# dist1ll/pomcpp

Measured on NVIDIA B200. Metric: env-steps/sec, higher is better.
Workload: dtype u8/int32

## Files before the change

pomcpp_b200/csrc/pom_batch.cu:

```cuda
#include <cuda_runtime.h>
#include <cstdio>
#include <cstdlib>
#include <cstring>
#include <fstream>
#include <sched.h>
#include <string>
#include <vector>
#include <new>

#include "pom_batch.h"
#include "pom_kernels.cuh"

namespace
{

thread_local std::string g_err;

int fail(int code, const char* what, cudaError_t ce = cudaSuccess)
{
    g_err = what;
    if(ce != cudaSuccess)
    {
        g_err += ": ";
        g_err += cudaGetErrorString(ce);
// ... 9 lines not shown
};

#define CK(expr) do { cudaError_t ce_ = (expr); if(ce_ != cudaSuccess) return fail(POM_E_CUDA, #expr, ce_); } while(0)

constexpr uint64_t TILE_ALIGN = 256;
constexpr uint64_t XFER_CHUNK = 65536;
constexpr size_t   FLUSH_BYTES = size_t(256) << 20;

}

struct pom_batch {
    int       device = 0;
    uint64_t  n_envs = 0;
    uint64_t  n_alloc = 0;
    uint64_t  env_offset = 0;
    uint32_t  n_templates = 0;
    uint32_t  max_ticks = 0;
    int       tpb = 128;
    int       n_sms = 1;
    int       ws_nw = 20;
    uint32_t  attr_ws = 0;
    uint32_t  walk = 0;
    int       pingpong = 1;
    int       no_spec = 0;
    int       policy_pertick = 1;
    int       obs_fused = 0;
    int       step_kernel = 0;
    bool      teams = false;
    int       policy_view = -1;
    uint8_t*  recs = nullptr;
    uint8_t*  templates = nullptr;
    uint32_t* episodes = nullptr;
    unsigned long long* stats = nullptr;
    uint32_t* moves_buf = nullptr;
    uint8_t*  status_buf = nullptr;
    pom_state* aos_stage = nullptr;
    uint8_t*  st_stage = nullptr;
    uint32_t* bad_count = nullptr;
    uint32_t* fin_counter = nullptr;
    uint32_t* policy = nullptr;
    void*     flush_buf = nullptr;
    uint32_t* idx_buf = nullptr;
    uint64_t  idx_cap = 0;
    cudaEvent_t ev_expand = nullptr;
    cudaStream_t stream = nullptr;
    cudaEvent_t ev[2] = { nullptr, nullptr };
    static constexpr int MAX_CHUNKS = 16;
    cudaStream_t s_h2d = nullptr, s_d2h = nullptr, s_k2 = nullptr;
    cudaEvent_t ev_k2 = nullptr;
    cudaEvent_t ev_in[MAX_CHUNKS] = {}, ev_done[MAX_CHUNKS] = {}, ev_out = nullptr, ev_begin = nullptr;
    std::vector<int32_t> seeds;
    uint64_t  launches = 0;
    bool      forked = false;
    uint32_t  attr_done = 0;

    pomk::BatchParams params() const
    {
        pomk::BatchParams P;
        P.recs = recs; P.n_envs = n_envs; P.env_offset = env_offset; P.templates = templates;
        P.n_templates = n_templates; P.max_ticks = max_ticks;
        P.tmpl_mask = (n_templates & (n_templates - 1u)) == 0u ? n_templates - 1u : 0u; P.episodes = episodes; P.stats = stats;
        P.policy = policy; P.policy_stride = n_alloc;
        return P;
    }
};

namespace
{

int use(const pom_batch* cb, bool join = true)
{
    if(!cb) return fail(POM_E_ARG, "null handle");
    CK(cudaSetDevice(cb->device));
    pom_batch* b = const_cast<pom_batch*>(cb);
    if(join && b->forked)
    {
        CK(cudaEventRecord(b->ev_k2, b->s_k2));
        CK(cudaStreamWaitEvent(b->stream, b->ev_k2, 0));
        b->forked = false;
    }
    return POM_OK;
}

enum { ATTR_STEP = 1, ATTR_ROLLOUT = 2, ATTR_ROLLOUT_POLICY = 4, ATTR_POLICY_MOVES = 8, ATTR_EXPAND = 16, ATTR_OBS = 32, ATTR_ROLLOUT_SPEC = 64, ATTR_OBS_CROPPED = 128 };
constexpr uint32_t attr_bit(uint32_t which, bool teams, bool fog = false) { return (fog ? which << 16 : which) << (teams ? 8 : 0); }

uint32_t policy_view_bits(const pom_batch* b)
{
    return uint32_t(b->policy_view > 15 ? 15 : b->policy_view) << pomk::POLICY_VIEW_SHIFT;
}

template<typename K>
int set_smem(pom_batch* b, uint32_t which, K kernel, uint32_t bytes)
{
    if(b->attr_done & which) return POM_OK;
    CK(cudaFuncSetAttribute(kernel, cudaFuncAttributeMaxDynamicSharedMemorySize, int(bytes)));
    b->attr_done |= which;
    return POM_OK;
}

int ensure_stage(pom_batch* b)
{
    if(!b->aos_stage)
    {
        CK(cudaMalloc(&b->aos_stage, XFER_CHUNK * sizeof(pom_state)));
        CK(cudaMalloc(&b->st_stage, XFER_CHUNK));
        CK(cudaMalloc(&b->bad_count, sizeof(uint32_t)));
    }
    return POM_OK;
}

int ensure_policy(pom_batch* b)
{
    if(!b->policy)
    {
        CK(cudaMalloc(&b->policy, 9 * b->n_alloc * sizeof(uint32_t)));
        CK(cudaMemsetAsync(b->policy, 0, 9 * b->n_alloc * sizeof(uint32_t), b->stream));
    }
    return POM_OK;
}

int fill_from_templates(pom_batch* b)
{
    const uint64_t words = b->n_envs * POM_REC_WORDS;
    pomk::k_fill_from_templates<<<unsigned((words + 255) / 256), 256, 0, b->stream>>>(b->params());
    b->launches++;
    CK(cudaGetLastError());
// ... 31 lines not shown
            b->launches++;
            CK(cudaGetLastError());
            CK(cudaStreamSynchronize(b->stream));
            b->seeds.resize(n);
            for(uint32_t k = 0; k < n; k++) b->seeds[k] = first_seed + int32_t(idx[k]);
            return POM_OK;
        }
    }
    return fail(POM_E_ARG, "could not find enough clean seeds");
}

int pack_into(pom_batch* b, uint8_t* dst_recs, uint64_t first, uint64_t count, const pom_state* states, const uint8_t* status, uint32_t* bad_total)
{
    int rc = ensure_stage(b);
    if(rc) return rc;
    for(uint64_t done = 0; done < count; done += XFER_CHUNK)
    {
        const uint64_t c = count - done < XFER_CHUNK ? count - done : XFER_CHUNK;
        CK(cudaMemcpyAsync(b->aos_stage, states + done, c * sizeof(pom_state), cudaMemcpyHostToDevice, b->stream));
        if(status) CK(cudaMemcpyAsync(b->st_stage, status + done, c, cudaMemcpyHostToDevice, b->stream));
        CK(cudaMemsetAsync(b->bad_count, 0, sizeof(uint32_t), b->stream));
        pomk::k_pack<<<unsigned((c + 127) / 128), 128, 0, b->stream>>>(b->aos_stage, status ? b->st_stage : nullptr, dst_recs, first + done, c, b->bad_count);
        b->launches++;
        CK(cudaGetLastError());
        uint32_t bad = 0;
        CK(cudaMemcpyAsync(&bad, b->bad_count, sizeof(uint32_t), cudaMemcpyDeviceToHost, b->stream));
        CK(cudaStreamSynchronize(b->stream));
        *bad_total += bad;
    }
    return POM_OK;
}

constexpr int WS_NW = 20, WS_NBUF = 24;

template<int NW, bool OBS, bool FREEZE = false, bool SPEC = false, bool TEAMS = false>
int launch_step_ws(pom_batch* b, const pomk::BatchParams& P, const pomk::StepIO& io, uint32_t flags, cudaStream_t on)
{
    typedef pomk::RingScratch<WS_NBUF> R;
    const uint32_t bit = TEAMS ? (1u << (24 + (FREEZE ? 2 : (OBS ? 1 : 0)))) :
                         SPEC ? 2u : (FREEZE ? 1u : (1u << (NW + (OBS ? 1 : 0))));
    if(!(b->attr_ws & bit))
    {
        CK(cudaFuncSetAttribute(pomk::k_step_ws<NW, WS_NBUF, OBS, FREEZE, SPEC, TEAMS>, cudaFuncAttributeMaxDynamicSharedMemorySize, int(R::BYTES)));
        b->attr_ws |= bit;
    }
    const uint64_t n_slices = (P.n_envs + 31) / 32;
    const unsigned grid = unsigned(n_slices < uint64_t(b->n_sms) ? n_slices : uint64_t(b->n_sms));
    pomk::k_step_ws<NW, WS_NBUF, OBS, FREEZE, SPEC, TEAMS><<<grid, (NW + 1) * 32, R::BYTES, on ? on : b->stream>>>(P, io, flags);
    b->launches++;
    CK(cudaGetLastError());
    return POM_OK;
}

int launch_step_io(pom_batch* b, const pomk::BatchParams& P, pomk::StepIO io, uint32_t flags, cudaStream_t on)
{
    io.bulk = (reinterpret_cast<uintptr_t>(io.moves) & 15u) == 0u ? 1u : 0u;
    if(P.n_envs == b->n_envs && b->pingpong) io.reverse = (b->walk++) & 1u;
    if(b->teams)
    {
        if(flags & pomk::STEP_FREEZE_TRUNCATED) return launch_step_ws<WS_NW, false, true, false, true>(b, P, io, flags, on);
        if(io.obs) return launch_step_ws<WS_NW, true, false, false, true>(b, P, io, flags, on);
        return launch_step_ws<WS_NW, false, false, false, true>(b, P, io, flags, on);
    }
    if(flags & pomk::STEP_FREEZE_TRUNCATED) return launch_step_ws<WS_NW, false, true>(b, P, io, flags, on);
    if(b->ws_nw == WS_NW && (flags & ~uint32_t(POM_STEP_OVERLAP)) == uint32_t(POM_STEP_AUTORESET | POM_STEP_COUNT) && io.bulk &&
       !io.status_out && !io.obs && !io.joint && !io.done_bits && !io.fin_env && !b->no_spec)
        return launch_step_ws<WS_NW, false, false, true>(b, P, io, flags, on);
    if(io.obs) return launch_step_ws<WS_NW, true>(b, P, io, flags, on);
    switch(b->ws_nw)
    {
    case 12: return launch_step_ws<12, false>(b, P, io, flags, on);
    case 14: return launch_step_ws<14, false>(b, P, io, flags, on);
    case 16: return launch_step_ws<16, false>(b, P, io, flags, on);
    case 18: return launch_step_ws<18, false>(b, P, io, flags, on);
    case 22: return launch_step_ws<22, false>(b, P, io, flags, on);
    default: return launch_step_ws<WS_NW, false>(b, P, io, flags, on);
    }
}

template<int TPB, bool TEAMS = false>
int launch_step(pom_batch* b, const uint8_t* moves_dev, uint32_t flags, uint8_t* status_dev, uint64_t first = 0, uint64_t count = 0, cudaStream_t on = nullptr,
                bool tile_kernel = false)
{
    pomk::BatchParams P = b->params();
    if(count)
    {
        P.recs += first * POM_REC_BYTES; P.episodes += first; P.env_offset += first; P.n_envs = count;
        moves_dev += 4 * first;
        if(status_dev) status_dev += first;
    }
    if(b->step_kernel == 0 && !tile_kernel)
    {
        pomk::StepIO io{};
        io.moves = moves_dev;
        io.status_out = status_dev;
        return launch_step_io(b, P, io, flags, on);
    }
    { int rc = set_smem(b, attr_bit(ATTR_STEP, TEAMS), pomk::k_step<TPB, TEAMS>, pomk::TileScratch<TPB>::BYTES); if(rc) return rc; }
    const unsigned grid = unsigned((P.n_envs + TPB - 1) / TPB);
    pomk::k_step<TPB, TEAMS><<<grid, TPB, pomk::TileScratch<TPB>::BYTES, on ? on : b->stream>>>(P, reinterpret_cast<const uint32_t*>(moves_dev), flags, status_dev);
    b->launches++;
    CK(cudaGetLastError());
    return POM_OK;
}

template<int TPB, bool TEAMS = false, bool FOG = false>
// ... 121 lines not shown
    } while(0)
#define POM_DISPATCH_MODE(h, fn, ...) \
    do { \
        if((h)->teams) return fn<128, true>(__VA_ARGS__); \
        POM_DISPATCH(h, fn, __VA_ARGS__); \
    } while(0)
#define POM_DISPATCH_POLICY(h, fn, ...) \
    do { \
        if((h)->policy_view >= 0) \
        { \
            if((h)->teams) return fn<128, true, true>(__VA_ARGS__); \
            return fn<128, false, true>(__VA_ARGS__); \
        } \
        POM_DISPATCH_MODE(h, fn, __VA_ARGS__); \
    } while(0)

extern "C" {

const char* pom_last_error(void) { return g_err.c_str(); }

int pom_device_count(void)
{
    int n = 0;
    if(cudaGetDeviceCount(&n) != cudaSuccess) { cudaGetLastError(); return 0; }
    return n;
}

int pom_batch_init(pom_batch** out, int device, uint64_t n_envs, const pom_init_desc* desc)
{
    if(!out || !desc || n_envs == 0 || desc->n_templates == 0) return fail(POM_E_ARG, "pom_batch_init: bad argument");
    if(n_envs > (uint64_t(1) << 31)) return fail(POM_E_ARG, "pom_batch_init: too many envs for one handle");
    int ndev = 0;
    cudaError_t ce = cudaGetDeviceCount(&ndev);
    if(ce != cudaSuccess || ndev == 0) return fail(POM_E_CUDA, "no CUDA device: the step path has no CPU fallback", ce);
    if(device < 0 || device >= ndev) return fail(POM_E_ARG, "pom_batch_init: no such device");
    CK(cudaSetDevice(device));
    pom_batch* b = new(std::nothrow) pom_batch();
    if(!b) return fail(POM_E_NOMEM, "host allocation failed");
    b->device = device;
    b->n_envs = n_envs;
    b->n_alloc = (n_envs + TILE_ALIGN - 1) / TILE_ALIGN * TILE_ALIGN;
    b->env_offset = desc->env_offset;
    b->n_templates = desc->n_templates;
    b->max_ticks = desc->max_ticks;
    b->teams = (desc->flags & POM_INIT_TEAMS) != 0;
    cudaDeviceGetAttribute(&b->n_sms, cudaDevAttrMultiProcessorCount, device);
    if(b->n_sms < 1) b->n_sms = 1;
    if(const char* e = std::getenv("POM_STEP_KERNEL")) b->step_kernel = std::strcmp(e, "tile") == 0 ? 1 : 0;
    if(const char* e = std::getenv("POM_WS_NW")) b->ws_nw = std::atoi(e);
    if(const char* e = std::getenv("POM_STEP_PINGPONG")) b->pingpong = std::atoi(e) != 0;
    if(const char* e = std::getenv("POM_OBS_FUSED")) b->obs_fused = std::atoi(e) != 0;
    if(const char* e = std::getenv("POM_WS_NOSPEC")) b->no_spec = std::atoi(e) != 0;
    if(const char* e = std::getenv("POM_ROLL_POLICY")) b->policy_pertick = std::strcmp(e, "fused") != 0;
    if(const char* e = std::getenv("POM_TPB"))
    {
        const int t = std::atoi(e);
        if(t == 32 || t == 64 || t == 128 || t == 256) b->tpb = t;
    }
    int rc = POM_OK;
    do {
        if(cudaStreamCreateWithFlags(&b->stream, cudaStreamNonBlocking) != cudaSuccess ||
           cudaEventCreate(&b->ev[0]) != cudaSuccess || cudaEventCreate(&b->ev[1]) != cudaSuccess ||
           cudaStreamCreateWithFlags(&b->s_h2d, cudaStreamNonBlocking) != cudaSuccess ||
           cudaStreamCreateWithFlags(&b->s_d2h, cudaStreamNonBlocking) != cudaSuccess ||
           cudaStreamCreateWithFlags(&b->s_k2, cudaStreamNonBlocking) != cudaSuccess ||
           cudaEventCreateWithFlags(&b->ev_k2, cudaEventDisableTiming) != cudaSuccess ||
           cudaEventCreateWithFlags(&b->ev_out, cudaEventDisableTiming) != cudaSuccess ||
           cudaEventCreateWithFlags(&b->ev_begin, cudaEventDisableTiming) != cudaSuccess)
        { rc = fail(POM_E_CUDA, "stream/event creation failed", cudaGetLastError()); break; }
        if(cudaMalloc(&b->recs, b->n_alloc * POM_REC_BYTES) != cudaSuccess ||
           cudaMalloc(&b->templates, size_t(b->n_templates) * POM_REC_BYTES) != cudaSuccess ||
           cudaMalloc(&b->episodes, b->n_alloc * sizeof(uint32_t)) != cudaSuccess ||
           cudaMalloc(&b->stats, POM_STATS_WORDS * sizeof(unsigned long long)) != cudaSuccess ||
           cudaMalloc(&b->moves_buf, b->n_alloc * 4) != cudaSuccess ||
           cudaMalloc(&b->status_buf, b->n_alloc) != cudaSuccess)
        { rc = fail(POM_E_NOMEM, "device allocation failed", cudaGetLastError()); break; }
        if(cudaMemsetAsync(b->recs, 0, b->n_alloc * POM_REC_BYTES, b->stream) != cudaSuccess ||
           cudaMemsetAsync(b->episodes, 0, b->n_alloc * sizeof(uint32_t), b->stream) != cudaSuccess ||
           cudaMemsetAsync(b->stats, 0, POM_STATS_WORDS * sizeof(unsigned long long), b->stream) != cudaSuccess)
        { rc = fail(POM_E_CUDA, "memset failed", cudaGetLastError()); break; }
        if(desc->host_templates)
        {
            uint32_t bad = 0;
            rc = pack_into(b, b->templates, 0, b->n_templates, desc->host_templates, nullptr, &bad);
            if(rc) break;
            if(bad) { rc = fail(POM_E_STATE, "a host template cannot be represented in the packed record"); break; }
        }
        else
        {
            rc = build_templates_from_seeds(b, desc->first_seed);
            if(rc) break;
        }
        if(!(desc->flags & POM_INIT_EMPTY))
        {
            rc = fill_from_templates(b);
            if(rc) break;
        }
        if(cudaStreamSynchronize(b->stream) != cudaSuccess) { rc = fail(POM_E_CUDA, "init sync failed", cudaGetLastError()); break; }
    } while(0);
    if(rc) { pom_batch_destroy(b); return rc; }
    *out = b;
    return POM_OK;
}

int pom_batch_destroy(pom_batch* b)
{
    if(!b) return POM_OK;
    cudaSetDevice(b->device);
    if(b->s_k2) cudaStreamSynchronize(b->s_k2);
    if(b->stream) cudaStreamSynchronize(b->stream);
    cudaFree(b->recs); cudaFree(b->templates); cudaFree(b->episodes); cudaFree(b->stats);
    cudaFree(b->moves_buf); cudaFree(b->status_buf); cudaFree(b->aos_stage); cudaFree(b->st_stage);
    cudaFree(b->bad_count); cudaFree(b->flush_buf); cudaFree(b->idx_buf); if(b->ev_expand) cudaEventDestroy(b->ev_expand); cudaFree(b->policy); cudaFree(b->fin_counter);
    if(b->ev[0]) cudaEventDestroy(b->ev[0]);
    if(b->ev[1]) cudaEventDestroy(b->ev[1]);
    for(int i = 0; i < pom_batch::MAX_CHUNKS; i++) { if(b->ev_in[i]) cudaEventDestroy(b->ev_in[i]); if(b->ev_done[i]) cudaEventDestroy(b->ev_done[i]); }
    if(b->ev_out) cudaEventDestroy(b->ev_out);
    if(b->ev_begin) cudaEventDestroy(b->ev_begin);
    if(b->s_h2d) cudaStreamDestroy(b->s_h2d);
    if(b->s_d2h) cudaStreamDestroy(b->s_d2h);
    if(b->s_k2) cudaStreamDestroy(b->s_k2);
    if(b->ev_k2) cudaEventDestroy(b->ev_k2);
    if(b->stream) cudaStreamDestroy(b->stream);
    delete b;
    return POM_OK;
}

int pom_batch_sync(pom_batch* b)
{
    int rc = use(b); if(rc) return rc;
    CK(cudaStreamSynchronize(b->stream));
    return POM_OK;
}

int pom_batch_upload(pom_batch* b, uint64_t first, uint64_t count, const pom_state* states, const uint8_t* status)
{
    int rc = use(b); if(rc) return rc;
    if(!states) return fail(POM_E_ARG, "pom_batch_upload: null states");
    if(first > b->n_envs || count > b->n_envs - first) return fail(POM_E_RANGE, "pom_batch_upload: range outside the batch");
    uint32_t bad = 0;
    rc = pack_into(b, b->recs, first, count, states, status, &bad);
    if(rc) return rc;
    if(bad) return fail(POM_E_STATE, "pom_batch_upload: some states cannot be represented (marked POM_STATUS_INVALID)");
    return POM_OK;
}

int pom_batch_download(pom_batch* b, uint64_t first, uint64_t count, pom_state* states, uint8_t* status)
{
    int rc = use(b); if(rc) return rc;
    if(first > b->n_envs || count > b->n_envs - first) return fail(POM_E_RANGE, "pom_batch_download: range outside the batch");
    rc = ensure_stage(b); if(rc) return rc;
    for(uint64_t done = 0; done < count; done += XFER_CHUNK)
    {
        const uint64_t c = count - done < XFER_CHUNK ? count - done : XFER_CHUNK;
        pomk::k_unpack<<<unsigned((c + 127) / 128), 128, 0, b->stream>>>(b->recs, states ? b->aos_stage : nullptr, b->st_stage, first + done, c);
        b->launches++;
        CK(cudaGetLastError());
        if(states) CK(cudaMemcpyAsync(states + done, b->aos_stage, c * sizeof(pom_state), cudaMemcpyDeviceToHost, b->stream));
        if(status) CK(cudaMemcpyAsync(status + done, b->st_stage, c, cudaMemcpyDeviceToHost, b->stream));
        CK(cudaStreamSynchronize(b->stream));
    }
    return POM_OK;
}

int pom_batch_observe(pom_batch* b, uint64_t first, uint64_t count, int agent, int view, pom_state* states, uint8_t* status)
// ... 17 lines not shown
}

uint64_t pom_batch_obs_stride(const pom_batch* b) { return b ? b->n_alloc : 0; }

int pom_batch_observe_planes(pom_batch* b, uint8_t* obs_dev, uint32_t agent_mask, int view)
{
    int rc = use(b); if(rc) return rc;
    if(!obs_dev) return fail(POM_E_ARG, "pom_batch_observe_planes: null output");
    if(agent_mask == 0 || agent_mask > 0xFu || view < 0) return fail(POM_E_ARG, "pom_batch_observe_planes: agent_mask must be 1..15 and view >= 0");
    POM_DISPATCH(b, launch_observe_planes, b, obs_dev, agent_mask, view);
}

int pom_device_copy(int device, void* dst, const void* src, uint64_t bytes)
{
    if(!dst || !src) return fail(POM_E_ARG, "pom_device_copy: null pointer");
    CK(cudaSetDevice(device));
    CK(cudaMemcpy(dst, src, bytes, cudaMemcpyDefault));
    return POM_OK;
}

int pom_batch_reset(pom_batch* b)
{
    int rc = use(b); if(rc) return rc;
    CK(cudaMemsetAsync(b->episodes, 0, b->n_alloc * sizeof(uint32_t), b->stream));
    CK(cudaMemsetAsync(b->stats, 0, POM_STATS_WORDS * sizeof(unsigned long long), b->stream));
    if(b->policy) CK(cudaMemsetAsync(b->policy, 0, 9 * b->n_alloc * sizeof(uint32_t), b->stream));
    return fill_from_templates(b);
}

int pom_batch_templates(pom_batch* b, pom_state* out, int32_t* seeds_out)
{
    int rc = use(b); if(rc) return rc;
    if(!out) return fail(POM_E_ARG, "pom_batch_templates: null output");
    rc = ensure_stage(b); if(rc) return rc;
    for(uint64_t done = 0; done < b->n_templates; done += XFER_CHUNK)
    {
        const uint64_t c = b->n_templates - done < XFER_CHUNK ? b->n_templates - done : XFER_CHUNK;
        pomk::k_unpack<<<unsigned((c + 127) / 128), 128, 0, b->stream>>>(b->templates, b->aos_stage, b->st_stage, done, c);
        b->launches++;
        CK(cudaGetLastError());
        CK(cudaMemcpyAsync(out + done, b->aos_stage, c * sizeof(pom_state), cudaMemcpyDeviceToHost, b->stream));
        CK(cudaStreamSynchronize(b->stream));
    }
    if(seeds_out)
    {
        for(uint32_t k = 0; k < b->n_templates; k++) seeds_out[k] = k < b->seeds.size() ? b->seeds[k] : 0;
    }
    return POM_OK;
}

int pom_batch_step(pom_batch* b, const uint8_t* moves_dev, uint32_t flags)
{
    const bool overlap = (flags & POM_STEP_OVERLAP) && b && b->n_envs >= (uint64_t(1) << 18);
    int rc = use(b, !overlap); if(rc) return rc;
    if(!moves_dev) return fail(POM_E_ARG, "pom_batch_step: null moves");
    if(!overlap) POM_DISPATCH_MODE(b, launch_step, b, moves_dev, flags, nullptr);
    static int parts = -1;
    if(parts < 0) { const char* e = std::getenv("POM_STEP_PARTS"); parts = e ? std::atoi(e) : 2; if(parts < 2 || parts > 16) parts = 2; }
    const uint64_t per = ((b->n_envs + parts - 1) / parts + 1023) / 1024 * 1024;
    const bool tile_parts = b->n_envs <= (uint64_t(1) << 19) && !b->no_spec;
    CK(cudaEventRecord(b->ev_begin, b->stream));
    CK(cudaStreamWaitEvent(b->s_k2, b->ev_begin, 0));
    int c = 0;
    for(uint64_t first = 0; first < b->n_envs; first += per, c++)
    {
        const uint64_t count = first + per <= b->n_envs ? per : b->n_envs - first;
        rc = [&]() -> int { POM_DISPATCH_MODE(b, launch_step, b, moves_dev, flags, nullptr, first, count, (c & 1) ? b->s_k2 : b->stream, tile_parts); }();
        if(rc) return rc;
    }
    b->forked = true;
    return POM_OK;
}

static int enqueue_step_pipeline(pom_batch* b, const uint8_t* moves_host, uint8_t* status_host, uint32_t flags, int chunks, uint64_t per)
{
    const uint64_t n = b->n_envs;
    CK(cudaEventRecord(b->ev_begin, b->stream));
    CK(cudaStreamWaitEvent(b->s_h2d, b->ev_begin, 0));
    if(chunks > 1) CK(cudaStreamWaitEvent(b->s_k2, b->ev_begin, 0));
    for(int c = 0; c < chunks; c++)
    {
        const uint64_t first = uint64_t(c) * per, count = (first + per <= n) ? per : n - first;
        cudaStream_t compute = (c & 1) ? b->s_k2 : b->stream;
        CK(cudaMemcpyAsync(reinterpret_cast<uint8_t*>(b->moves_buf) + 4 * first, moves_host + 4 * first, 4 * count, cudaMemcpyHostToDevice, b->s_h2d));
        CK(cudaEventRecord(b->ev_in[c], b->s_h2d));
        CK(cudaStreamWaitEvent(compute, b->ev_in[c], 0));
        const int rc = [&]() -> int { POM_DISPATCH_MODE(b, launch_step, b, reinterpret_cast<const uint8_t*>(b->moves_buf), flags,
                                                   status_host ? b->status_buf : nullptr, first, count, compute); }();
        if(rc) return rc;
        if(status_host)
        {
            CK(cudaEventRecord(b->ev_done[c], compute));
            CK(cudaStreamWaitEvent(b->s_d2h, b->ev_done[c], 0));
            CK(cudaMemcpyAsync(status_host + first, b->status_buf + first, count, cudaMemcpyDeviceToHost, b->s_d2h));
        }
    }
    if(chunks > 1)
    {
        CK(cudaEventRecord(b->ev_k2, b->s_k2));
        CK(cudaStreamWaitEvent(b->stream, b->ev_k2, 0));
    }
    if(status_host)
    {
        CK(cudaEventRecord(b->ev_out, b->s_d2h));
        CK(cudaStreamWaitEvent(b->stream, b->ev_out, 0));
    }
    return POM_OK;
}

// ... 488 lines not shown
```

pomcpp_b200/csrc/pom_kernels.cuh:

```cuda
#ifndef POM_KERNELS_CUH_
#define POM_KERNELS_CUH_

#include <cuda_runtime.h>
#include <stdint.h>
#include "pom_core.cuh"
#include "pom_policy.cuh"
#include "pom_batch.h"

namespace pomk
{

constexpr uint32_t STEP_FREEZE_TRUNCATED = 0x40000000u;

enum { ST_STEPS = 0, ST_EPISODES = 1, ST_WIN0 = 2, ST_DRAWS = 6, ST_TRUNC = 7, ST_SUMLEN = 8, ST_INVALID = 9 };

struct BatchParams {
    uint8_t*            recs;
    uint64_t            n_envs;
    uint64_t            env_offset;
    const uint8_t*      templates;
    uint32_t            n_templates;
    uint32_t            tmpl_mask;
    uint32_t            max_ticks;
    uint32_t*           episodes;
// ... 1 lines not shown
    uint32_t*           policy;
    uint64_t            policy_stride;
};

__device__ __forceinline__ uint32_t smem_u32(const void* p) { return uint32_t(__cvta_generic_to_shared(p)); }

__device__ __forceinline__ void mbar_init(uint64_t* bar, uint32_t count)
{
    asm volatile("mbarrier.init.shared::cta.b64 [%0], %1;" :: "r"(smem_u32(bar)), "r"(count));
}
__device__ __forceinline__ void fence_barrier_init()
{
    asm volatile("fence.mbarrier_init.release.cluster;" ::: "memory");
}
__device__ __forceinline__ void fence_proxy_async()
{
    asm volatile("fence.proxy.async.shared::cta;" ::: "memory");
}
__device__ __forceinline__ void mbar_expect_tx(uint64_t* bar, uint32_t bytes)
{
    asm volatile("mbarrier.arrive.expect_tx.shared::cta.b64 _, [%0], %1;" :: "r"(smem_u32(bar)), "r"(bytes) : "memory");
}
__device__ __forceinline__ void mbar_arrive(uint64_t* bar)
{
    asm volatile("mbarrier.arrive.shared::cta.b64 _, [%0];" :: "r"(smem_u32(bar)) : "memory");
}
__device__ __forceinline__ void mbar_wait(uint64_t* bar, uint32_t parity)
{
    asm volatile(
        "{\n"
        ".reg .pred p;\n"
        "WAIT_LOOP:\n"
        "mbarrier.try_wait.parity.shared::cta.b64 p, [%0], %1;\n"
        "@p bra WAIT_DONE;\n"
        "bra WAIT_LOOP;\n"
        "WAIT_DONE:\n"
        "}\n" :: "r"(smem_u32(bar)), "r"(parity) : "memory");
}
__device__ __forceinline__ void bulk_g2s(void* smem_dst, const void* gmem_src, uint32_t bytes, uint64_t* bar)
{
    asm volatile("cp.async.bulk.shared::cluster.global.mbarrier::complete_tx::bytes [%0], [%1], %2, [%3];"
                 :: "r"(smem_u32(smem_dst)), "l"(gmem_src), "r"(bytes), "r"(smem_u32(bar)) : "memory");
}
__device__ __forceinline__ void bulk_s2g(void* gmem_dst, const void* smem_src, uint32_t bytes)
{
    asm volatile("cp.async.bulk.global.shared::cta.bulk_group [%0], [%1], %2;"
                 :: "l"(gmem_dst), "r"(smem_u32(smem_src)), "r"(bytes) : "memory");
    asm volatile("cp.async.bulk.commit_group;" ::: "memory");
}
__device__ __forceinline__ void bulk_wait_read_all()
{
    asm volatile("cp.async.bulk.wait_group.read 0;" ::: "memory");
}

__device__ __forceinline__ void warp_add(unsigned long long* dst, uint32_t v)
{
    const uint32_t s = __reduce_add_sync(0xFFFFFFFFu, v);
    if((threadIdx.x & 31u) == 0u && s) atomicAdd(dst, (unsigned long long)s);
}

struct EpisodeAcc {
    uint32_t fin_draw = 0u;
    uint32_t trunc_abort = 0u;
    uint32_t win01 = 0u, win23 = 0u;
    uint32_t len = 0u;
    uint32_t steps = 0u;
    uint32_t pending = 0u;
};

__device__ __forceinline__ void acc_add(EpisodeAcc& A, bool fin, uint32_t status, uint32_t len)
{
    if(!fin) return;
    const bool done = (status & POM_STATUS_DONE) != 0u;
    const bool draw = done && (status & POM_STATUS_DRAW);
    const bool trunc = !done && (status & POM_STATUS_TRUNCATED);
    const uint32_t w = (status & POM_STATUS_WINNER_MASK) >> POM_STATUS_WINNER_SHIFT;
    A.fin_draw += 1u + (draw ? 0x10000u : 0u);
    A.trunc_abort += (trunc ? 1u : 0u) + ((!done && !trunc) ? 0x10000u : 0u);
    if(done && !draw)
    {
        const uint32_t inc = (w & 1u) ? 0x10000u : 1u;
        if(w & 2u) A.win23 += inc; else A.win01 += inc;
    }
    A.len += len;
    A.pending++;
}

__device__ __forceinline__ void acc_flush(unsigned long long* stats, EpisodeAcc& A, bool count_steps)
{
    const uint32_t lane = threadIdx.x & 31u;
    if(__reduce_or_sync(0xFFFFFFFFu, A.pending))
    {
        const uint32_t v[9] = { A.fin_draw & 0xFFFFu, A.win01 & 0xFFFFu, A.win01 >> 16, A.win23 & 0xFFFFu, A.win23 >> 16,
                                A.fin_draw >> 16, A.trunc_abort & 0xFFFFu, A.len, A.trunc_abort >> 16 };
#pragma unroll
        for(int k = 0; k < 9; k++)
        {
            const uint32_t sum = __reduce_add_sync(0xFFFFFFFFu, v[k]);
            if(lane == 0u && sum) atomicAdd(stats + 1 + k, (unsigned long long)sum);
        }
    }
    if(count_steps)
    {
        const uint32_t sum = __reduce_add_sync(0xFFFFFFFFu, A.steps);
        if(lane == 0u && sum) atomicAdd(stats + ST_STEPS, (unsigned long long)sum);
    }
// ... 203 lines not shown
template<int TPB, bool TEAMS = false>
__global__ void __launch_bounds__(TPB) k_step(BatchParams P, const uint32_t* __restrict__ moves, uint32_t flags, uint8_t* __restrict__ status_out)
{
    extern __shared__ __align__(128) uint8_t smem[];
    const uint64_t env = uint64_t(blockIdx.x) * TPB + threadIdx.x;
    const bool active = env < P.n_envs;
    const bool raw = (flags & POM_STEP_RAW) != 0u;

    constexpr uint32_t SLICE_BYTES = 32 * POM_REC_BYTES;
    const uint32_t warp = threadIdx.x >> 5, lane = threadIdx.x & 31u;
    uint64_t* bar = reinterpret_cast<uint64_t*>(smem + TileScratch<TPB>::OFF_BAR) + warp;
    uint8_t* sslice = smem + warp * SLICE_BYTES;
    uint8_t* gslice = P.recs + (size_t(blockIdx.x) * TPB + warp * 32u) * POM_REC_BYTES;
    if(lane == 0)
    {
        mbar_init(bar, 1);
        fence_barrier_init();
        mbar_expect_tx(bar, SLICE_BYTES);
        bulk_g2s(sslice, gslice, SLICE_BYTES, bar);
    }
    const uint32_t m = active ? __ldg(moves + env) : 0u;
    uint32_t ep_now = (active && (flags & POM_STEP_AUTORESET)) ? P.episodes[env] : 0u;
    __syncwarp();
    mbar_wait(bar, 0);

    uint8_t* rec = sslice + lane * POM_REC_BYTES;
    const bool stepped = active && !(rec[R_STATUS] & (raw ? POM_STATUS_INVALID : (POM_STATUS_DONE | POM_STATUS_INVALID)));
    warp_tick<TEAMS>(sslice, rec, m, stepped, raw, smem + TileScratch<TPB>::OFF_LIST + 8u * warp,
                     (flags & POM_STEP_CONTINUE_UNDEFINED) ? pomcore::F_INVALID_MASK_CONTINUE : pomcore::F_INVALID_MASK);
    EpisodeAcc acc;
    acc.steps = stepped ? 1u : 0u;
    uint32_t st_end = active ? rec[R_STATUS] : 0u;
    if(flags & POM_STEP_AUTORESET)
    {
        const uint32_t st = finish_and_reset(sslice, rec, P, env, active && stepped, true, ep_now, acc);
        if(active && stepped) st_end = st;
    }
    acc_flush(P.stats, acc, (flags & POM_STEP_COUNT) != 0u);
    if(status_out && active) status_out[env] = uint8_t(st_end);
    fence_proxy_async();
    __syncwarp();
    if(lane == 0)
    {
        bulk_s2g(gslice, sslice, SLICE_BYTES);
        bulk_wait_read_all();
    }
}

struct StepIO {
    const void* moves;
    uint32_t    joint;
    uint32_t    bulk;
    uint32_t    reverse;
    uint8_t*    status_out;
    uint32_t*   done_bits;
    uint32_t*   fin_env;
    uint8_t*    fin_status;
    uint32_t*   fin_counter;
    uint32_t*   fin_count_out;
    uint32_t    fin_capacity;
    uint8_t*    obs;
    uint64_t    obs_stride;
    uint32_t    obs_mask;
    int         obs_view;
};

__device__ __forceinline__ uint32_t moves_of_joint(uint32_t j)
{
    const uint32_t a0 = j % 6u, r1 = j / 6u, a1 = r1 % 6u, r2 = r1 / 6u, a2 = r2 % 6u, a3 = (r2 / 6u) % 6u;
    return a0 | (a1 << 8) | (a2 << 16) | (a3 << 24);
}

template<int NBUF> struct RingScratch {
    static constexpr uint32_t SLICE_BYTES = 32 * POM_REC_BYTES;
    static constexpr uint32_t SLOT = SLICE_BYTES + 128 + 16;
    static constexpr uint32_t OFF_FULL = NBUF * SLOT;
    static constexpr uint32_t MAIL = 256;
    static constexpr uint32_t OFF_MAIL = OFF_FULL + 8 * NBUF;
    static constexpr uint32_t OFF_TICKET = OFF_MAIL + 4 * MAIL;
    static constexpr uint32_t FIN_CAP = 480;
    static constexpr uint32_t OFF_FIN = OFF_TICKET + 16;
    static constexpr uint32_t OFF_FIN_ENV = OFF_FIN + 16;
    static constexpr uint32_t OFF_FIN_ST = OFF_FIN_ENV + 4 * FIN_CAP;
    static constexpr uint32_t BYTES = OFF_FIN_ST + FIN_CAP;
};

template<int NW, int NBUF, bool OBS, bool FREEZE, bool SPEC = false, bool TEAMS = false>
__global__ void __launch_bounds__((NW + 1) * 32, 1) k_step_ws(BatchParams P, StepIO io_in, uint32_t flags_in)
{
    const uint32_t flags = SPEC ? uint32_t(POM_STEP_AUTORESET | POM_STEP_COUNT) : flags_in;
    StepIO io = io_in;
    if(SPEC)
    {
        io.joint = 0u; io.bulk = 1u; io.status_out = nullptr; io.obs = nullptr; io.done_bits = nullptr; io.fin_env = nullptr;
    }
    const uint32_t* __restrict__ moves = static_cast<const uint32_t*>(io.moves);
    const uint16_t* __restrict__ joint = static_cast<const uint16_t*>(io.moves);
    uint8_t* __restrict__ status_out = io.status_out;
    const uint32_t moves_bulk = io.bulk;
    const uint32_t mv_bytes = io.joint ? 64u : 128u;
    extern __shared__ __align__(128) uint8_t smem[];
    typedef RingScratch<NBUF> R;
    uint64_t* full = reinterpret_cast<uint64_t*>(smem + R::OFF_FULL);
    volatile uint32_t* mail = reinterpret_cast<volatile uint32_t*>(smem + R::OFF_MAIL);
    uint32_t* ticket = reinterpret_cast<uint32_t*>(smem + R::OFF_TICKET);
    uint32_t* free_mask = ticket + 2;
    const uint32_t warp = threadIdx.x >> 5, lane = threadIdx.x & 31u;
    const uint64_t n_slices = (P.n_envs + 31u) / 32u;
    const uint32_t T = blockIdx.x < n_slices ? uint32_t((n_slices - blockIdx.x + gridDim.x - 1u) / gridDim.x) : 0u;
    if(threadIdx.x == 0)
    {
        for(int b = 0; b < NBUF; b++) mbar_init(full + b, 1);
        ticket[0] = 0u;
        ticket[1] = 0u;
        *free_mask = (NBUF >= 32) ? 0xFFFFFFFFu : ((1u << NBUF) - 1u);
        reinterpret_cast<uint32_t*>(smem + R::OFF_FIN)[0] = 0u;
        reinterpret_cast<uint32_t*>(smem + R::OFF_FIN)[1] = 0xFFFFFFFFu;
        fence_barrier_init();
    }
    for(uint32_t i = threadIdx.x; i < R::MAIL; i += blockDim.x) mail[i] = 0u;
    __syncthreads();

    if(warp == NW)
    {
        if(lane != 0) return;
        uint32_t parity = 0u;
        for(uint32_t t = 0; t < T; t++)
        {
            uint32_t fm;
            while((fm = *reinterpret_cast<volatile uint32_t*>(free_mask)) == 0u) __nanosleep(40);
            const uint32_t b = uint32_t(__ffs(int(fm))) - 1u;
            atomicAnd(free_mask, ~(1u << b));
            const uint64_t s0 = blockIdx.x + uint64_t(t) * gridDim.x;
            const uint64_t s = io.reverse ? n_slices - 1u - s0 : s0;
            const bool whole = (s + 1u) * 32u <= P.n_envs;
            const uint32_t mbytes = (moves_bulk && whole) ? mv_bytes : 0u;
            mbar_expect_tx(full + b, R::SLICE_BYTES + mbytes);
            bulk_g2s(smem + b * R::SLOT, P.recs + s * R::SLICE_BYTES, R::SLICE_BYTES, full + b);
            if(mbytes) bulk_g2s(smem + b * R::SLOT + R::SLICE_BYTES, static_cast<const uint8_t*>(io.moves) + s * mv_bytes, mbytes, full + b);
            mail[t % R::MAIL] = ((t + 1u) << 8) | (b << 1) | ((parity >> b) & 1u);
            parity ^= 1u << b;
        }
        return;
    }

    const bool raw = (flags & POM_STEP_RAW) != 0u;
    EpisodeAcc acc;
    for(;;)
    {
        uint32_t t = 0u;
        if(lane == 0) t = atomicAdd(ticket, 1u);
        t = __shfl_sync(FULL_WARP, t, 0);
        if(t >= T) break;
        const uint64_t s0 = blockIdx.x + uint64_t(t) * gridDim.x;
        const uint64_t s = io.reverse ? n_slices - 1u - s0 : s0;
        const uint64_t env = s * 32u + lane;
        const bool active = env < P.n_envs;
        const bool whole = (s + 1u) * 32u <= P.n_envs;
        uint32_t m = 0u;
        if(!(moves_bulk && whole) && active) m = io.joint ? uint32_t(__ldg(joint + env)) : __ldg(moves + env);
        uint32_t ep_now = (active && (flags & POM_STEP_AUTORESET)) ? P.episodes[env] : 0u;
        uint32_t v;
        while(((v = mail[t % R::MAIL]) >> 8) != t + 1u) __nanosleep(20);
        const uint32_t b = (v >> 1) & 31u;
        uint8_t* sslice = smem + b * R::SLOT;
        mbar_wait(full + b, v & 1u);
        if(moves_bulk && whole)
            m = io.joint ? uint32_t(reinterpret_cast<const uint16_t*>(sslice + R::SLICE_BYTES)[lane])
                         : reinterpret_cast<const uint32_t*>(sslice + R::SLICE_BYTES)[lane];
        if(io.joint) m = moves_of_joint(m);

        uint8_t* rec = sslice + lane * POM_REC_BYTES;
        const bool stepped = active && !(rec[R_STATUS] & ((raw ? POM_STATUS_INVALID : (POM_STATUS_DONE | POM_STATUS_INVALID)) |
                                                          (FREEZE ? POM_STATUS_TRUNCATED : 0)));
        warp_tick<TEAMS>(sslice, rec, m, stepped, raw, sslice + R::SLICE_BYTES + 128u,
                         (flags & POM_STEP_CONTINUE_UNDEFINED) ? pomcore::F_INVALID_MASK_CONTINUE : pomcore::F_INVALID_MASK);
        acc.steps += stepped ? 1u : 0u;
        uint32_t st_end = active ? rec[R_STATUS] : 0u;
        if(flags & POM_STEP_AUTORESET)
        {
            const uint32_t st = finish_and_reset(sslice, rec, P, env, active && stepped, true, ep_now, acc);
            if(active && stepped) st_end = st;
        }
        if(status_out && active) status_out[env] = uint8_t(st_end);
        if(io.done_bits || io.fin_env)
        {
            const bool ended = active && stepped && (st_end & (POM_STATUS_DONE | POM_STATUS_TRUNCATED | POM_STATUS_INVALID)) != 0u;
            const uint32_t em = __ballot_sync(FULL_WARP, ended);
            if(io.done_bits && lane == 0) io.done_bits[s] = em;
            if(io.fin_env && em)
            {
                uint32_t* fin = reinterpret_cast<uint32_t*>(smem + R::OFF_FIN);
                const uint32_t k = uint32_t(__popc(em));
                uint32_t pos = 0u;
                if(lane == 0) pos = atomicAdd(fin, k);
                pos = __shfl_sync(FULL_WARP, pos, 0);
                const uint32_t mine = uint32_t(__popc(em & ((1u << lane) - 1u)));
                if(pos + k <= R::FIN_CAP)
                {
                    if(ended)
                    {
                        reinterpret_cast<uint32_t*>(smem + R::OFF_FIN_ENV)[pos + mine] = uint32_t(env);
                        smem[R::OFF_FIN_ST + pos + mine] = uint8_t(st_end);
                    }
                }
                else
                {
                    if(lane == 0) { atomicMin(fin + 1, pos); pos = atomicAdd(io.fin_counter, k); }
                    pos = __shfl_sync(FULL_WARP, pos, 0) + mine;
                    if(ended && pos < io.fin_capacity)
                    {
                        io.fin_env[pos] = uint32_t(env);
                        io.fin_status[pos] = uint8_t(st_end);
                    }
                }
            }
        }
        fence_proxy_async();
        __syncwarp();
        if(lane == 0) bulk_s2g(P.recs + s * R::SLICE_BYTES, sslice, R::SLICE_BYTES);
        if(OBS && io.obs)
        {
            const uint32_t n_valid = whole ? 32u : uint32_t(P.n_envs - s * 32u);
            uint32_t k = 0u;
            for(int a = 0; a < 4; a++)
            {
                if(!((io.obs_mask >> a) & 1u)) continue;
                warp_observe_slice(sslice, a, io.obs_view, io.obs + (uint64_t(k) * io.obs_stride + s * 32u) * POM_OBS_BYTES, n_valid);
                k++;
            }
        }
        __syncwarp();
        if(lane == 0)
        {
            bulk_wait_read_all();
            __threadfence_block();
            atomicOr(free_mask, 1u << b);
        }
        __syncwarp();
    }
    acc_flush(P.stats, acc, (flags & POM_STEP_COUNT) != 0u);
    if(io.fin_env)
    {
        __threadfence_block();
        uint32_t* warps_done = ticket + 1;
        bool last = false;
        if(lane == 0) last = atomicAdd(warps_done, 1u) == uint32_t(NW - 1);
        last = __shfl_sync(FULL_WARP, last ? 1 : 0, 0) != 0;
        if(last)
        {
            __threadfence_block();
            const volatile uint32_t* fin = reinterpret_cast<const volatile uint32_t*>(smem + R::OFF_FIN);
            const uint32_t k = fin[1] != 0xFFFFFFFFu ? fin[1] : fin[0];
            unsigned long long old = 0ull;
            if(lane == 0) old = atomicAdd(reinterpret_cast<unsigned long long*>(io.fin_counter), (1ull << 32) | k);
            old = __shfl_sync(FULL_WARP, old, 0);
            const uint32_t base = uint32_t(old);
            for(uint32_t i = lane; i < k; i += 32u)
            {
                if(base + i < io.fin_capacity)
                {
                    io.fin_env[base + i] = reinterpret_cast<const uint32_t*>(smem + R::OFF_FIN_ENV)[i];
                    io.fin_status[base + i] = smem[R::OFF_FIN_ST + i];
                }
            }
            if(lane == 0 && uint32_t(old >> 32) == gridDim.x - 1u)
            {
                const uint32_t count = base + k;
                *io.fin_count_out = count < io.fin_capacity ? count : io.fin_capacity;
                *reinterpret_cast<volatile unsigned long long*>(io.fin_counter) = 0ull;
            }
        }
    }
}

struct GlobalAgentStore {
    uint32_t* base;
    uint64_t  stride;
    __device__ __forceinline__ pompolicy::SimpleSt load(int a) const
    {
        pompolicy::SimpleSt s;
        s.w0 = base[uint64_t(2 * a) * stride];
        s.w1 = base[uint64_t(2 * a + 1) * stride];
        return s;
    }
    __device__ __forceinline__ void store(int a, const pompolicy::SimpleSt& v)
    {
        base[uint64_t(2 * a) * stride] = v.w0;
        base[uint64_t(2 * a + 1) * stride] = v.w1;
    }
    __device__ __forceinline__ void clear(uint32_t episode)
    {
#pragma unroll
        for(int k = 0; k < 8; k++) base[uint64_t(k) * stride] = 0u;
// ... 368 lines not shown
```

Before: 10.00 billion.

## Chain consecutive step kernels with PDL and per-slice sequence flags

Adds a chained step path for large batches. Each step kernel is launched with programmatic dependent launch, so the next step's grid can start before the previous one finishes. Correctness is kept by per-slice sequence counters written with release stores after the bulk store completes, and the producer warp spins on them with acquire loads before loading a slice. The chained variant also uses a smaller mailbox and no fin buffer so two CTAs fit per SM. This removes kernel launch and tail bubbles between steps, at the cost of spin-waiting and extra global flag traffic.

Result: slower. 9.129 billion, median of 6 (-8.7%).

```diff
diff --git a/pomcpp_b200/csrc/pom_batch.cu b/pomcpp_b200/csrc/pom_batch.cu
--- a/pomcpp_b200/csrc/pom_batch.cu
+++ b/pomcpp_b200/csrc/pom_batch.cu
@@ -85,6 +85,10 @@
     std::vector<int32_t> seeds;
     uint64_t  launches = 0;
     bool      forked = false;
+    bool      chain = false;
+    bool      chained = false;
+    uint32_t  chain_seq = 0;
+    uint32_t* slice_seq = nullptr;
     uint32_t  attr_done = 0;
 
     pomk::BatchParams params() const
@@ -106,6 +110,7 @@
     if(!cb) return fail(POM_E_ARG, "null handle");
     CK(cudaSetDevice(cb->device));
     pom_batch* b = const_cast<pom_batch*>(cb);
+    b->chained = false;
     if(join && b->forked)
     {
         CK(cudaEventRecord(b->ev_k2, b->s_k2));
@@ -243,6 +248,61 @@
     return POM_OK;
 }
 
+constexpr int CHAIN_NW = 10, CHAIN_NBUF = 12;
+constexpr uint64_t CHAIN_MIN_ENVS = uint64_t(1) << 19;
+static_assert(pomk::ws_ctas_per_sm<CHAIN_NBUF, true>() == 2, "two chained CTAs must fit one SM");
+
+template<bool SPEC, bool TEAMS, int NW = CHAIN_NW, int NBUF = CHAIN_NBUF>
+int launch_step_chain(pom_batch* b, pomk::StepIO io, uint32_t flags, bool follows)
+{
+    typedef pomk::RingScratch<NBUF, true> R;
+    auto kernel = pomk::k_step_ws<NW, NBUF, false, false, SPEC, TEAMS, true>;
+    const uint32_t bit = NW != CHAIN_NW ? (1u << 30) : 1u << (27 + (TEAMS ? 2 : (SPEC ? 1 : 0)));
+    if(!(b->attr_ws & bit))
+    {
+        CK(cudaFuncSetAttribute(kernel, cudaFuncAttributeMaxDynamicSharedMemorySize, int(R::BYTES)));
+        b->attr_ws |= bit;
+    }
+    if(++b->chain_seq == 0u) { b->chain_seq = 1u; follows = false; }
+    io.seq = b->chain_seq;
+    io.wait_for = follows ? b->chain_seq - 1u : 0u;
+    io.done_bits = b->slice_seq;
+    io.reverse = 0u;
+    b->walk += 1u + (b->walk & 1u);
+    const pomk::BatchParams P = b->params();
+    const uint64_t n_slices = (P.n_envs + 31) / 32, ctas = pomk::ws_ctas_per_sm<NBUF, true>() * uint64_t(b->n_sms);
+    cudaLaunchConfig_t cfg = {};
+    cfg.gridDim = dim3(unsigned(n_slices < ctas ? n_slices : ctas));
+    cfg.blockDim = dim3((NW + 1) * 32);
+    cfg.dynamicSmemBytes = R::BYTES;
+    cfg.stream = b->stream;
+    cudaLaunchAttribute attr[1];
+    attr[0].id = cudaLaunchAttributeProgrammaticStreamSerialization;
+    attr[0].val.programmaticStreamSerializationAllowed = 1;
+    cfg.attrs = attr;
+#ifdef CHX_NOPDL
+    cfg.numAttrs = 0;
+#else
+    cfg.numAttrs = follows ? 1 : 0;
+#endif
+    CK(cudaLaunchKernelEx(&cfg, kernel, P, io, flags));
+    b->launches++;
+    b->chained = true;
+    return POM_OK;
+}
+
+int step_chain(pom_batch* b, const uint8_t* moves_dev, uint32_t flags, bool follows)
+{
+    pomk::StepIO io{};
+    io.moves = moves_dev;
+    io.bulk = (reinterpret_cast<uintptr_t>(moves_dev) & 15u) == 0u ? 1u : 0u;
+    if(b->teams) return launch_step_chain<false, true>(b, io, flags, follows);
+    if(std::getenv("POM_CHAIN_ONE") && std::atoi(std::getenv("POM_CHAIN_ONE")))    return launch_step_chain<true, false, WS_NW, WS_NBUF>(b, io, flags, follows);
+    if((flags & ~uint32_t(POM_STEP_OVERLAP)) == uint32_t(POM_STEP_AUTORESET | POM_STEP_COUNT) && io.bulk && !b->no_spec)
+        return launch_step_chain<true, false>(b, io, flags, follows);
+    return launch_step_chain<false, false>(b, io, flags, follows);
+}
+
 int launch_step_io(pom_batch* b, const pomk::BatchParams& P, pomk::StepIO io, uint32_t flags, cudaStream_t on)
 {
     io.bulk = (reinterpret_cast<uintptr_t>(io.moves) & 15u) == 0u ? 1u : 0u;
@@ -470,6 +530,7 @@
     if(const char* e = std::getenv("POM_OBS_FUSED")) b->obs_fused = std::atoi(e) != 0;
     if(const char* e = std::getenv("POM_WS_NOSPEC")) b->no_spec = std::atoi(e) != 0;
     if(const char* e = std::getenv("POM_ROLL_POLICY")) b->policy_pertick = std::strcmp(e, "fused") != 0;
+    if(const char* e = std::getenv("POM_STEP_CHAIN")) b->chain = std::atoi(e) != 0; else b->chain = true;
     if(const char* e = std::getenv("POM_TPB"))
     {
         const int t = std::atoi(e);
@@ -491,10 +552,12 @@
            cudaMalloc(&b->episodes, b->n_alloc * sizeof(uint32_t)) != cudaSuccess ||
            cudaMalloc(&b->stats, POM_STATS_WORDS * sizeof(unsigned long long)) != cudaSuccess ||
            cudaMalloc(&b->moves_buf, b->n_alloc * 4) != cudaSuccess ||
+           cudaMalloc(&b->slice_seq, b->n_alloc / 32 * sizeof(uint32_t)) != cudaSuccess ||
            cudaMalloc(&b->status_buf, b->n_alloc) != cudaSuccess)
         { rc = fail(POM_E_NOMEM, "device allocation failed", cudaGetLastError()); break; }
         if(cudaMemsetAsync(b->recs, 0, b->n_alloc * POM_REC_BYTES, b->stream) != cudaSuccess ||
            cudaMemsetAsync(b->episodes, 0, b->n_alloc * sizeof(uint32_t), b->stream) != cudaSuccess ||
+           cudaMemsetAsync(b->slice_seq, 0, b->n_alloc / 32 * sizeof(uint32_t), b->stream) != cudaSuccess ||
            cudaMemsetAsync(b->stats, 0, POM_STATS_WORDS * sizeof(unsigned long long), b->stream) != cudaSuccess)
         { rc = fail(POM_E_CUDA, "memset failed", cudaGetLastError()); break; }
         if(desc->host_templates)
@@ -514,6 +577,16 @@
             rc = fill_from_templates(b);
             if(rc) break;
         }
+        if(b->chain)
+        {
+            typedef pomk::RingScratch<CHAIN_NBUF, true> R;
+            auto kernel = pomk::k_step_ws<CHAIN_NW, CHAIN_NBUF, false, false, true, false, true>;
+            int per_sm = 0;
+            if(cudaFuncSetAttribute(kernel, cudaFuncAttributeMaxDynamicSharedMemorySize, int(R::BYTES)) != cudaSuccess ||
+               cudaOccupancyMaxActiveBlocksPerMultiprocessor(&per_sm, kernel, (CHAIN_NW + 1) * 32, R::BYTES) != cudaSuccess)
+            { rc = fail(POM_E_CUDA, "chained step kernel", cudaGetLastError()); break; }
+            b->chain = per_sm == 2;
+        }
         if(cudaStreamSynchronize(b->stream) != cudaSuccess) { rc = fail(POM_E_CUDA, "init sync failed", cudaGetLastError()); break; }
     } while(0);
     if(rc) { pom_batch_destroy(b); return rc; }
@@ -528,7 +601,7 @@
     if(b->s_k2) cudaStreamSynchronize(b->s_k2);
     if(b->stream) cudaStreamSynchronize(b->stream);
     cudaFree(b->recs); cudaFree(b->templates); cudaFree(b->episodes); cudaFree(b->stats);
-    cudaFree(b->moves_buf); cudaFree(b->status_buf); cudaFree(b->aos_stage); cudaFree(b->st_stage);
+    cudaFree(b->moves_buf); cudaFree(b->status_buf); cudaFree(b->slice_seq); cudaFree(b->aos_stage); cudaFree(b->st_stage);
     cudaFree(b->bad_count); cudaFree(b->flush_buf); cudaFree(b->idx_buf); if(b->ev_expand) cudaEventDestroy(b->ev_expand); cudaFree(b->policy); cudaFree(b->fin_counter);
     if(b->ev[0]) cudaEventDestroy(b->ev[0]);
     if(b->ev[1]) cudaEventDestroy(b->ev[1]);
@@ -652,9 +725,11 @@
 int pom_batch_step(pom_batch* b, const uint8_t* moves_dev, uint32_t flags)
 {
     const bool overlap = (flags & POM_STEP_OVERLAP) && b && b->n_envs >= (uint64_t(1) << 18);
+    const bool follows = b && b->chained;
     int rc = use(b, !overlap); if(rc) return rc;
     if(!moves_dev) return fail(POM_E_ARG, "pom_batch_step: null moves");
     if(!overlap) POM_DISPATCH_MODE(b, launch_step, b, moves_dev, flags, nullptr);
+    if(b->chain && b->n_envs > CHAIN_MIN_ENVS && b->step_kernel == 0 && b->ws_nw == WS_NW) return step_chain(b, moves_dev, flags, follows);
     static int parts = -1;
     if(parts < 0) { const char* e = std::getenv("POM_STEP_PARTS"); parts = e ? std::atoi(e) : 2; if(parts < 2 || parts > 16) parts = 2; }
     const uint64_t per = ((b->n_envs + parts - 1) / parts + 1023) / 1024 * 1024;
diff --git a/pomcpp_b200/csrc/pom_kernels.cuh b/pomcpp_b200/csrc/pom_kernels.cuh
--- a/pomcpp_b200/csrc/pom_kernels.cuh
+++ b/pomcpp_b200/csrc/pom_kernels.cuh
@@ -77,6 +77,37 @@
 {
     asm volatile("cp.async.bulk.wait_group.read 0;" ::: "memory");
 }
+__device__ __forceinline__ void bulk_wait_all()
+{
+    asm volatile("cp.async.bulk.wait_group 0;" ::: "memory");
+}
+__device__ __forceinline__ void bulk_wait_group_1()
+{
+    asm volatile("cp.async.bulk.wait_group 1;" ::: "memory");
+}
+
+__device__ __forceinline__ void fence_proxy_async_global()
+{
+    asm volatile("fence.proxy.async.global;" ::: "memory");
+}
+__device__ __forceinline__ uint32_t ld_acquire_gpu(const uint32_t* p)
+{
+    uint32_t v;
+    asm volatile("ld.acquire.gpu.global.u32 %0, [%1];" : "=r"(v) : "l"(p) : "memory");
+    return v;
+}
+__device__ __forceinline__ void st_release_gpu(uint32_t* p, uint32_t v)
+{
+    asm volatile("st.release.gpu.global.u32 [%0], %1;" :: "l"(p), "r"(v) : "memory");
+}
+__device__ __forceinline__ void pdl_launch_dependents()
+{
+    asm volatile("griddepcontrol.launch_dependents;" ::: "memory");
+}
+__device__ __forceinline__ void pdl_wait_prerequisite()
+{
+    asm volatile("griddepcontrol.wait;" ::: "memory");
+}
 
 __device__ __forceinline__ void warp_add(unsigned long long* dst, uint32_t v)
 {
@@ -386,6 +417,7 @@
     uint32_t    joint;
     uint32_t    bulk;
     uint32_t    reverse;
+    uint32_t    seq;
     uint8_t*    status_out;
     uint32_t*   done_bits;
     uint32_t*   fin_env;
@@ -393,6 +425,7 @@
     uint32_t*   fin_counter;
     uint32_t*   fin_count_out;
     uint32_t    fin_capacity;
+    uint32_t    wait_for;
     uint8_t*    obs;
     uint64_t    obs_stride;
     uint32_t    obs_mask;
@@ -405,36 +438,50 @@
     return a0 | (a1 << 8) | (a2 << 16) | (a3 << 24);
 }
 
-template<int NBUF> struct RingScratch {
+template<int NBUF, bool CHAIN = false> struct RingScratch {
     static constexpr uint32_t SLICE_BYTES = 32 * POM_REC_BYTES;
     static constexpr uint32_t SLOT = SLICE_BYTES + 128 + 16;
     static constexpr uint32_t OFF_FULL = NBUF * SLOT;
-    static constexpr uint32_t MAIL = 256;
+#ifdef CHX_MAIL64
+    static constexpr uint32_t MAIL = 64;
+#else
+    static constexpr uint32_t MAIL = CHAIN ? 64 : 256;
+#endif
     static constexpr uint32_t OFF_MAIL = OFF_FULL + 8 * NBUF;
     static constexpr uint32_t OFF_TICKET = OFF_MAIL + 4 * MAIL;
-    static constexpr uint32_t FIN_CAP = 480;
+    static constexpr uint32_t FIN_CAP = CHAIN ? 0 : 480;
     static constexpr uint32_t OFF_FIN = OFF_TICKET + 16;
     static constexpr uint32_t OFF_FIN_ENV = OFF_FIN + 16;
     static constexpr uint32_t OFF_FIN_ST = OFF_FIN_ENV + 4 * FIN_CAP;
     static constexpr uint32_t BYTES = OFF_FIN_ST + FIN_CAP;
 };
 
-template<int NW, int NBUF, bool OBS, bool FREEZE, bool SPEC = false, bool TEAMS = false>
-__global__ void __launch_bounds__((NW + 1) * 32, 1) k_step_ws(BatchParams P, StepIO io_in, uint32_t flags_in)
-{
+constexpr uint32_t CHAIN_CTA_SMEM = 115712;
+template<int NBUF, bool CHAIN> constexpr int ws_ctas_per_sm() { return (CHAIN && RingScratch<NBUF, CHAIN>::BYTES <= CHAIN_CTA_SMEM) ? 2 : 1; }
+
+template<int NW, int NBUF, bool OBS, bool FREEZE, bool SPEC = false, bool TEAMS = false, bool CHAIN = false>
+__global__ void __launch_bounds__((NW + 1) * 32, (ws_ctas_per_sm<NBUF, CHAIN>())) k_step_ws(BatchParams P, StepIO io_in, uint32_t flags_in)
+{
+    static_assert(!(CHAIN && (OBS || FREEZE)), "the chained step has no observation output and no frozen truncation");
     const uint32_t flags = SPEC ? uint32_t(POM_STEP_AUTORESET | POM_STEP_COUNT) : flags_in;
     StepIO io = io_in;
-    if(SPEC)
+    if(SPEC && !CHAIN)
     {
         io.joint = 0u; io.bulk = 1u; io.status_out = nullptr; io.obs = nullptr; io.done_bits = nullptr; io.fin_env = nullptr;
     }
+    if(CHAIN)
+    {
+        if(SPEC) { io.joint = 0u; io.bulk = 1u; }
+        io.status_out = nullptr; io.fin_env = nullptr;
+    }
+    uint32_t* const slice_seq = io.done_bits;
     const uint32_t* __restrict__ moves = static_cast<const uint32_t*>(io.moves);
     const uint16_t* __restrict__ joint = static_cast<const uint16_t*>(io.moves);
     uint8_t* __restrict__ status_out = io.status_out;
     const uint32_t moves_bulk = io.bulk;
     const uint32_t mv_bytes = io.joint ? 64u : 128u;
     extern __shared__ __align__(128) uint8_t smem[];
-    typedef RingScratch<NBUF> R;
+    typedef RingScratch<NBUF, CHAIN> R;
     uint64_t* full = reinterpret_cast<uint64_t*>(smem + R::OFF_FULL);
     volatile uint32_t* mail = reinterpret_cast<volatile uint32_t*>(smem + R::OFF_MAIL);
     uint32_t* ticket = reinterpret_cast<uint32_t*>(smem + R::OFF_TICKET);
@@ -454,11 +501,14 @@
     }
     for(uint32_t i = threadIdx.x; i < R::MAIL; i += blockDim.x) mail[i] = 0u;
     __syncthreads();
+    if(CHAIN) pdl_launch_dependents();
 
     if(warp == NW)
     {
         if(lane != 0) return;
         uint32_t parity = 0u;
+        auto slice_of = [&](uint32_t t) { const uint64_t s0 = blockIdx.x + uint64_t(t) * gridDim.x; return io.reverse ? n_slices - 1u - s0 : s0; };
+        uint32_t seen = (CHAIN && io.wait_for && T) ? ld_acquire_gpu(slice_seq + slice_of(0u)) : 0u;
         for(uint32_t t = 0; t < T; t++)
         {
             uint32_t fm;
@@ -468,18 +518,30 @@
             const uint64_t s0 = blockIdx.x + uint64_t(t) * gridDim.x;
             const uint64_t s = io.reverse ? n_slices - 1u - s0 : s0;
             const bool whole = (s + 1u) * 32u <= P.n_envs;
+#ifdef CHX_NOSYNC
+            if(false)
+#else
+            if(CHAIN && io.wait_for)
+#endif
+            {
+                while(seen != io.wait_for) { __nanosleep(64); seen = ld_acquire_gpu(slice_seq + s); }
+                fence_proxy_async_global();
+            }
             const uint32_t mbytes = (moves_bulk && whole) ? mv_bytes : 0u;
             mbar_expect_tx(full + b, R::SLICE_BYTES + mbytes);
             bulk_g2s(smem + b * R::SLOT, P.recs + s * R::SLICE_BYTES, R::SLICE_BYTES, full + b);
             if(mbytes) bulk_g2s(smem + b * R::SLOT + R::SLICE_BYTES, static_cast<const uint8_t*>(io.moves) + s * mv_bytes, mbytes, full + b);
             mail[t % R::MAIL] = ((t + 1u) << 8) | (b << 1) | ((parity >> b) & 1u);
             parity ^= 1u << b;
+            if(CHAIN && io.wait_for && t + 1u < T) seen = ld_acquire_gpu(slice_seq + slice_of(t + 1u));
         }
         return;
     }
 
     const bool raw = (flags & POM_STEP_RAW) != 0u;
     EpisodeAcc acc;
+    constexpr uint64_t NO_SLICE = ~0ull;
+    uint64_t prev_s = NO_SLICE;
     for(;;)
     {
         uint32_t t = 0u;
@@ -493,12 +555,24 @@
         const bool whole = (s + 1u) * 32u <= P.n_envs;
         uint32_t m = 0u;
         if(!(moves_bulk && whole) && active) m = io.joint ? uint32_t(__ldg(joint + env)) : __ldg(moves + env);
-        uint32_t ep_now = (active && (flags & POM_STEP_AUTORESET)) ? P.episodes[env] : 0u;
+#if defined(CHX_EP_CG_BEFORE)
+        uint32_t ep_now = (!CHAIN && active && (flags & POM_STEP_AUTORESET)) ? __ldcg(P.episodes + env) : 0u;
+#elif defined(CHX_EP_CG_AFTER) || defined(CHX_EP_AFTER)
+        uint32_t ep_now = 0u;
+#else
+        uint32_t ep_now = (!CHAIN && active && (flags & POM_STEP_AUTORESET)) ? P.episodes[env] : 0u;
+#endif
         uint32_t v;
         while(((v = mail[t % R::MAIL]) >> 8) != t + 1u) __nanosleep(20);
         const uint32_t b = (v >> 1) & 31u;
         uint8_t* sslice = smem + b * R::SLOT;
         mbar_wait(full + b, v & 1u);
+        if(CHAIN && active && (flags & POM_STEP_AUTORESET)) ep_now = __ldcg(P.episodes + env);
+#if defined(CHX_EP_CG_AFTER)
+        if(!CHAIN && active && (flags & POM_STEP_AUTORESET)) ep_now = __ldcg(P.episodes + env);
+#elif defined(CHX_EP_AFTER)
+        if(!CHAIN && active && (flags & POM_STEP_AUTORESET)) ep_now = P.episodes[env];
+#endif
         if(moves_bulk && whole)
             m = io.joint ? uint32_t(reinterpret_cast<const uint16_t*>(sslice + R::SLICE_BYTES)[lane])
                          : reinterpret_cast<const uint32_t*>(sslice + R::SLICE_BYTES)[lane];
@@ -517,7 +591,7 @@
             if(active && stepped) st_end = st;
         }
         if(status_out && active) status_out[env] = uint8_t(st_end);
-        if(io.done_bits || io.fin_env)
+        if(!CHAIN && (io.done_bits || io.fin_env))
         {
             const bool ended = active && stepped && (st_end & (POM_STATUS_DONE | POM_STATUS_TRUNCATED | POM_STATUS_INVALID)) != 0u;
             const uint32_t em = __ballot_sync(FULL_WARP, ended);
@@ -570,10 +644,22 @@
             bulk_wait_read_all();
             __threadfence_block();
             atomicOr(free_mask, 1u << b);
-        }
-        __syncwarp();
-    }
+            if(CHAIN)
+            {
+#if defined(CHX_NOSYNC)
+#elif defined(CHX_NOFENCE)
+                if(prev_s != NO_SLICE) { bulk_wait_group_1(); *reinterpret_cast<volatile uint32_t*>(slice_seq + prev_s) = io.seq; }
+#else
+                if(prev_s != NO_SLICE) { bulk_wait_group_1(); fence_proxy_async_global(); st_release_gpu(slice_seq + prev_s, io.seq); }
+#endif
+                prev_s = s;
+            }
+        }
+        __syncwarp();
+    }
+    if(CHAIN && lane == 0 && prev_s != NO_SLICE) { bulk_wait_all(); fence_proxy_async_global(); st_release_gpu(slice_seq + prev_s, io.seq); }
     acc_flush(P.stats, acc, (flags & POM_STEP_COUNT) != 0u);
+    if(CHAIN) pdl_wait_prerequisite();
     if(io.fin_env)
     {
         __threadfence_block();
```
